# r-mafi/ClaraGenomicsAnalysis

Measured on AMD Instinct MI355X. Metric: POA windows/sec (consensus), higher is better.
Workload: dtype int16

## Files before the change

### claragenomicsanalysis_amd/csrc/poa_batch.cpp

```cpp
#include <claraparabricks/genomeworks/cudapoa/batch.hpp>
#include <claraparabricks/genomeworks/cudapoa/utils.hpp>

#include "gwamd_cudapoa.h"
#include "host_common.hpp"
#include "poa_batch_internal.hpp"
#include "poa_common.hpp"

#include <hip/hip_runtime.h>

#include <algorithm>
#include <cstdio>
#include <cstdlib>
#include <cstring>
#include <iomanip>
#include <sstream>
#include <string>

extern "C" hipError_t gwamd_internal_poa_launch(const gwamd::poa::Buffers* b, const gwamd::poa::Dims* d,
                                       const gwamd::poa::Scores* sc, int score_bits, int size_bits, int banded,
                                       int msa, hipStream_t stream);
extern "C" int gwamd_internal_poa_blocks_per_cu(const gwamd::poa::Dims* d, int score_bits, int size_bits, int banded,
                                                int msa);

namespace claraparabricks
// ... 458 lines not shown
        num_seqs_           = 0;
        next_scores_offset_ = 0;
        avail_scorebuf_     = scorebuf_alloc_;
        generated_          = false;
    }

    int32_t score_bits() const { return score_bits_; }
    int32_t size_bits() const { return size_bits_; }
    const gwamd::poa::Dims& dims() const { return dims_; }
    const std::vector<uint8_t>& host_cons() const { return h_cons_; }
    const std::vector<uint16_t>& host_cov() const { return h_cov_; }
    const std::vector<int32_t>& host_cons_len() const { return h_len_out_; }
    const std::vector<uint8_t>& host_status() const { return h_status_; }
    const std::vector<uint8_t>& host_msa() const { return h_msa_; }
    const std::vector<int32_t>& host_msa_len() const { return h_msa_len_; }
    const std::vector<uint8_t>& host_msa_status() const { return h_msa_status_; }
    const std::vector<uint8_t>& host_g_bases() const { return h_g_bases_; }
    const std::vector<uint16_t>& host_g_in_cnt() const { return h_g_in_cnt_; }
    const std::vector<int32_t>& host_g_in_e() const { return h_g_in_e_; }
    const std::vector<uint16_t>& host_g_in_w() const { return h_g_in_w_; }
    const std::vector<int32_t>& host_final_nodes() const { return h_final_nodes_; }
    int32_t window_num_seqs(int32_t w) const { return h_win_.as<const gwamd::poa::WindowDesc>()[w].num_seqs; }
    int8_t output_mask() const { return output_mask_; }
    int64_t device_bytes() const { return int64_t(d_slab_.n + d_codes_.n + d_seqs_.n + d_wts_.n + d_len_.n + d_off_.n + d_win_.n); }
    int32_t kernel_kind() const
    {
        return dims_.lds_kernel == 3 ? (dims_.band_ad ? 4 : 3) : (dims_.lds_kernel ? 2 : 1);
    }
    int32_t max_poas() const { return max_poas_; }
    int32_t max_sequence_size() const { return bs_.max_sequence_size; }
    int32_t slots() const { return slots_; }
    int32_t resident_slots() const { return blocks_per_cu_; }
    void set_spoa_accurate(bool on) { dims_.spoa_accurate = on ? 1 : 0; }
    bool spoa_accurate() const { return dims_.spoa_accurate != 0; }

    void get_phases(int64_t* out)
    {
        ScopedDevice dev(device_id_);
        if (poa_count_ == 0)
            return;
        GWAMD_HIP_CHECK(hipMemcpyAsync(out, bufs_.phase, size_t(poa_count_) * 8 * gwamd::poa::kPhases,
                                       hipMemcpyDeviceToHost, stream_));
        GWAMD_HIP_CHECK(hipStreamSynchronize(stream_));
    }

    void get_stats(int64_t* cells, int32_t* final_nodes)
    {
        ScopedDevice dev(device_id_);
        if (poa_count_ == 0)
            return;
        GWAMD_HIP_CHECK(hipMemcpyAsync(cells, bufs_.cells, size_t(poa_count_) * 8, hipMemcpyDeviceToHost, stream_));
        GWAMD_HIP_CHECK(hipMemcpyAsync(final_nodes, bufs_.final_nodes, size_t(poa_count_) * 4, hipMemcpyDeviceToHost,
                                       stream_));
        GWAMD_HIP_CHECK(hipStreamSynchronize(stream_));
    }

private:
    int64_t window_bytes(int sz, bool msa) const
    {
        const int64_t mn = dims_.max_nodes, E = gwamd::poa::kMaxEdges, S = dims_.max_seqs;
        int64_t b        = 0;
        b += align8(mn) + 4 * align8(mn * 2) + align8(mn * E * 2);
        b += 3 * align8(mn * E * sz) + 2 * align8(mn * sz);
        b += align8(dims_.max_consensus) + align8(int64_t(dims_.max_consensus) * 2) + 32;
        b += int64_t(S) * dims_.max_seq_len * 2 + S * 12;
        if (msa)
            b += align8(mn * E * S * 2) + align8(mn * E * 2) + align8(S * sz) +
                 align8(S * int64_t(dims_.max_consensus));
        return b;
    }

    int64_t slot_bytes(int sz, int sbytes) const
    {
        const int64_t mn = dims_.max_nodes;
        int64_t b        = 0;
        b += 2 * align8(int64_t(dims_.aln_cap) * sz);
        b += int64_t(dims_.score_rows) * dims_.score_stride * sbytes;
        if (dims_.lds_kernel)
            b += dims_.aux_stride;
        b += align8(mn * 4) + align8(mn * 4 * sz);
        return b;
    }

    void plan_lds_kernel()
    {
        dims_.lds_kernel = 0;
        const char* env  = gwamd::host::diag_env("GWAMD_POA_KERNEL");
        if (env && std::string(env) == "v1")
            return;
        if (banded_ || size_bits_ != 16 || (score_bits_ != 16 && score_bits_ != 32))
            return;
        const bool wide      = score_bits_ == 32;
        auto a16             = [](int64_t v) { return (v + 15) & ~int64_t(15); };
        int ring_rows        = 8;
        const int64_t read_b = a16(int64_t(dims_.max_seq_len) + 48);
        int cpl = 8, nw = 1;
        const int ms = dims_.max_seq_len;
        if (!wide && ms > 512)
            nw = 2;
        if (wide)
        {
            nw  = ms <= 512 ? 1 : (ms <= 1024 ? 2 : (ms <= 2048 ? 4 : 8));
            cpl = ms <= 4096 ? 8 : 16;
        }
        if (const char* sh = gwamd::host::diag_env("GWAMD_POA_LDS_SHAPE"))
        {
            int c = 0, n = 0;
            if (std::sscanf(sh, "%d,%d", &c, &n) == 2)
            {
                const bool known =
                    wide ? ((c == 8 && (n == 1 || n == 2 || n == 4 || n == 8)) || (c == 16 && n == 8))
                         : ((n == 1 && (c == 8 || c == 16 || c == 24 || c == 32)) || (c == 8 && n >= 2 && n <= 4) ||
                            (c == 16 && n == 4) || (c == 4 && n == 4));
                if (!known)
                    throw std::invalid_argument("GWAMD_POA_LDS_SHAPE: unsupported columns/waves pair");
                cpl = c, nw = n;
            }
        }
        const int ebytes     = wide ? 4 : 2;
        const int64_t add_b  = 5 * a16(dims_.max_seq_len + 16) + 2 * (int64_t(dims_.max_nodes) + dims_.max_seq_len);
        const int64_t tile_b = int64_t(gwamd::poa::kTileRows) * gwamd::poa::kTileCols + gwamd::poa::kTbRankBytes;
        const int64_t rec_b  = a16(int64_t(dims_.max_nodes + 2) * 4);
        const int64_t sh_b   = a16(wide ? gwamd::poa::kShBytesW(nw) : gwamd::poa::kShBytes(nw));
        auto ring_bytes      = [&](int rows) {
            return a16(std::max<int64_t>({int64_t(rows) * dims_.score_stride * ebytes, tile_b, add_b}));
        };
        int64_t ring_b       = ring_bytes(ring_rows);
        int64_t fixed        = read_b + ring_b + rec_b + sh_b;
        int64_t target       = 40960 - 16;
        if (wide)
        {
            int64_t chosen = 0;
            for (int64_t budget : {int64_t(81920 - 16), int64_t(163840 - 64)})
            {
                for (int rows : {8, 4})
                {
                    const int64_t rb = ring_bytes(rows);
                    const int64_t fx = read_b + rb + rec_b + sh_b;
                    if (fx + 2048 <= budget)
                    {
                        ring_rows = rows, ring_b = rb, fixed = fx, chosen = budget;
                        break;
                    }
                }
                if (chosen)
                    break;
            }
            if (!chosen)
                return;
            target = chosen;
        }
        int64_t xl_cap       = std::max<int64_t>(1024, (target - fixed) / 2);
        xl_cap               = std::min<int64_t>(xl_cap, 65535);
        int64_t total        = fixed + a16(xl_cap * 2);
        if (const char* pad = gwamd::host::diag_env("GWAMD_POA_LDS_PAD"))
            total += a16(std::atoi(pad));
        if (total > (wide ? 163840 - 64 : 65536))
            return;
        dims_.lds_kernel    = 1;
        dims_.tb_rank       = tb_rank_default();
        dims_.lds_ring_off  = int32_t(read_b);
        dims_.lds_ring_rows = ring_rows;
        dims_.lds_rec_off   = int32_t(read_b + ring_b);
        dims_.lds_xl_off    = int32_t(read_b + ring_b + rec_b);
        dims_.lds_xl_cap    = int32_t(xl_cap);
        dims_.lds_sh_off    = int32_t(read_b + ring_b + rec_b + a16(xl_cap * 2));
        dims_.lds_bytes     = int32_t(total);
        dims_.lds_cpl       = cpl;
        dims_.lds_waves     = nw;
        dims_.code_stride   = int32_t(a16(int64_t(dims_.max_seq_len) + 48));
        const int64_t code_b = int64_t(dims_.score_rows) * dims_.code_stride;
        const int64_t cr_b   = a16(int64_t(dims_.max_nodes + 2) * ebytes);
        dims_.aux_carry_off  = int32_t(code_b);
        dims_.aux_stride     = code_b + cr_b;
    }

public:
    static int tb_rank_default()
    {
        int above_bits = 0;
        if (const char* ab = gwamd::host::diag_env("GWAMD_TB_ABOVE"))
            above_bits = (std::min(std::max(std::atoi(ab), 0), 6) + 1) << 3;
        return tb_walk_bits() | above_bits;
    }
    static int diag_bits()
    {
        const char* r = gwamd::host::diag_env("GWAMD_TOPSORT_RING");
        const char* f = gwamd::host::diag_env("GWAMD_POA_FWD");
        const char* t = gwamd::host::diag_env("GWAMD_TOPSORT");
        const char* d = gwamd::host::diag_env("GWAMD_RACON");
        const char* c = gwamd::host::diag_env("GWAMD_CONSENSUS");
        const char* b = gwamd::host::diag_env("GWAMD_CONSENSUS_LDS_BYTES");
        const int cap = b ? std::min(std::max(std::atoi(b), 1), 65535) : 0;
        return ((r && std::atoi(r) != 0) ? 1 : 0) | ((f && std::string(f) == "v1") ? 2 : 0) |
               ((t && std::string(t) == "fifo") ? 4 : 0) | ((d && std::string(d) == "v1") ? 8 : 0) |
               ((c && std::string(c) == "hbm") ? 16 : 0) | int(uint32_t(cap) << 16);
    }
    static int tb_walk_bits()
    {
        const char* ev = gwamd::host::diag_env("GWAMD_TB_WALK");
        const std::string v = ev ? ev : "";
        if (v == "scalar")
            return 2;
        if (v == "rect")
            return 1;
        if (v == "scalar_rect")
            return 0;
        if (v == "strip32")
            return 7;
        if (v == "scalar_strip32")
            return 6;
        return 3;
    }

private:
    void plan_band_kernel()
    {
        if (!banded_ || dims_.lds_kernel)
            return;
        const char* env = gwamd::host::diag_env("GWAMD_POA_KERNEL");
        if (env && std::string(env) == "v1")
            return;
        const int bw = dims_.band_width;
        if (bw % 128 != 0 || bw < 128 || bw > 1024 || gap_ > 0)
            return;
        auto a16          = [](int64_t v) { return (v + 15) & ~int64_t(15); };
        const int cpl     = bw / 64;
        const int sbytes  = score_bits_ / 8;
        const int rowsz   = (bw + gwamd::poa::kBandPad + cpl + cpl - 1) / cpl * cpl;
        const int64_t ms  = dims_.max_seq_len, mn = dims_.max_nodes;
        const int64_t read_b  = a16(gwamd::poa::kReadGuard + ms + bw + 48);
        const int64_t sh_b    = 64;
        const int ring_rows   = gwamd::poa::band_ring_rows(cpl), tile_rows = gwamd::poa::band_tile_rows(cpl);
        const int64_t ring_b  = a16(int64_t(ring_rows) * rowsz * sbytes) + 4 * 256 * 4 + 1024 * 4;
        const int64_t tile_b  = a16(int64_t(tile_rows) * bw + 64 * 16 + 512 + gwamd::poa::kTbRankBytes);
        const int64_t flags_b = 2 * a16(mn + 2);
        const int64_t add_b   = 7 * a16(ms + 16) + a16(2 * (mn + ms + 16));
        const int64_t ad_b    = a16(int64_t(gwamd::poa::kAdRing) * rowsz * sbytes + gwamd::poa::kWave * sbytes) +
                             a16(mn / 8 + 64);
        const char* fwd_env   = gwamd::host::diag_env("GWAMD_BAND_FWD");
        const bool force_ad   = fwd_env && std::string(fwd_env) == "ad" && cpl <= 4;
        const bool no_ad      = fwd_env && std::string(fwd_env) == "row";
        const int64_t min_w   = std::max({ring_b, tile_b, flags_b, force_ad ? ad_b : int64_t(0)});
        const int64_t want_w  = std::max(min_w, add_b);
        const int64_t kStatic = 256;
        int64_t total         = 0;
        int chosen_per_cu     = 1;
        for (int per_cu : {4, 2, 1})
        {
            const int64_t budget = (163840 / per_cu - kStatic) & ~int64_t(15);
            if ((!force_ad && read_b + want_w + sh_b <= budget) || per_cu == 1)
            {
                total         = budget;
                chosen_per_cu = per_cu;
                break;
            }
        }
        const int64_t work = total - read_b - sh_b;
        if (work < min_w)
            return;
        dims_.lds_kernel     = 3;
        int ad_waves = gwamd::poa::kAdMaxWaves;
        if (const char* ev = gwamd::host::diag_env("GWAMD_BAND_AD_WAVES"))
            ad_waves = std::max(1, std::min(gwamd::poa::kAdMaxWaves, std::atoi(ev)));
        dims_.band_ad        = (!no_ad && cpl <= 4 && chosen_per_cu == 1 && work >= ad_b) ? ad_waves : 0;
        dims_.tb_rank        = tb_rank_default();
        dims_.lds_cpl        = cpl;
        dims_.lds_waves      = 1;
        dims_.lds_bytes      = int32_t(total);
        dims_.lds_ring_off   = int32_t(read_b);
        dims_.lds_ring_rows  = ring_rows;
        dims_.lds_work_bytes = int32_t(work);
        dims_.lds_sh_off     = int32_t(read_b + work);
        dims_.score_stride   = rowsz;
        dims_.code_stride    = bw;
        const int64_t rows   = dims_.score_rows;
        int64_t o            = a16(rows * bw);
// ... 572 lines not shown
                             int32_t* max_nodes)
{
    return guarded([&] {
        batch->impl->fetch_graphs();
        const int32_t n = batch->impl->get_total_poas();
        for (int32_t w = 0; w < n; w++)
        {
            status[w]    = int32_t(batch->impl->graph_status(w));
            num_nodes[w] = batch->impl->host_final_nodes()[w];
        }
        *bases      = batch->impl->host_g_bases().data();
        *in_count   = batch->impl->host_g_in_cnt().data();
        *in_edges   = batch->impl->host_g_in_e().data();
        *in_weights = batch->impl->host_g_in_w().data();
        *max_nodes  = batch->impl->dims().max_nodes;
        return 0;
    });
}

int32_t gwamd_poa_batch_id(const gwamd_poa_batch* batch) { return batch->impl->batch_id(); }

void gwamd_poa_reset(gwamd_poa_batch* batch) { batch->impl->reset(); }

int32_t gwamd_poa_get_stats(gwamd_poa_batch* batch, int64_t* cells, int32_t* final_nodes)
{
    return guarded([&] {
        batch->impl->get_stats(cells, final_nodes);
        return 0;
    });
}

int32_t gwamd_poa_get_phase_ticks(gwamd_poa_batch* batch, int64_t* ticks)
{
    return guarded([&] {
        batch->impl->get_phases(ticks);
        return int32_t(gwamd::poa::kPhases);
    });
}

int32_t gwamd_poa_get_types(const gwamd_poa_batch* batch, int32_t* score_bits, int32_t* size_bits)
{
    *score_bits = batch->impl->score_bits();
    *size_bits  = batch->impl->size_bits();
    return batch->impl->kernel_kind();
}

int32_t gwamd_poa_env_tuning(int32_t* tb_rank, int32_t* band_fwd, int32_t* force_v1, int32_t* diag)
{
    if (!tb_rank || !band_fwd || !force_v1 || !diag)
    {
        gwamd::host::last_error() = "gwamd_poa_env_tuning: NULL output";
        return GWAMD_E_INVALID_ARGUMENT;
    }
    *tb_rank            = claraparabricks::genomeworks::cudapoa::PoaBatch::tb_rank_default();
    const char* fwd     = gwamd::host::diag_env("GWAMD_BAND_FWD");
    *band_fwd           = !fwd ? 0 : (std::string(fwd) == "ad" ? 1 : (std::string(fwd) == "row" ? 2 : 0));
    const char* kern    = gwamd::host::diag_env("GWAMD_POA_KERNEL");
    *force_v1           = kern && std::string(kern) == "v1" ? 1 : 0;
    *diag               = claraparabricks::genomeworks::cudapoa::PoaBatch::diag_bits();
    return 0;
}

int32_t gwamd_poa_set_spoa_accurate(gwamd_poa_batch* batch, int32_t on)
{
    const int32_t was = batch->impl->spoa_accurate() ? 1 : 0;
    batch->impl->set_spoa_accurate(on != 0);
    return was;
}

int32_t gwamd_poa_get_capacity(const gwamd_poa_batch* batch, int64_t* device_bytes, int32_t* max_poas)
{
    *device_bytes = batch->impl->device_bytes();
    *max_poas     = batch->impl->max_poas();
    return 0;
}

int32_t gwamd_poa_get_grid(const gwamd_poa_batch* batch, int32_t* slots, int32_t* resident)
{
    *slots    = batch->impl->slots();
    *resident = batch->impl->resident_slots();
    return 0;
}

static size_t query_free_memory(uint64_t given)
{
    if (given != 0)
        return size_t(given);
    size_t free_mem = 0, total = 0;
    if (hipMemGetInfo(&free_mem, &total) != hipSuccess)
        throw std::runtime_error("hipMemGetInfo failed");
    return free_mem;
}

int64_t gwamd_poa_estimate_max_poas(int32_t max_seq_sz, int32_t max_seq_per_poa, int32_t band_width, int32_t banded,
                                    int32_t msa, uint64_t free_device_memory, float quota, int32_t mismatch,
                                    int32_t gap, int32_t match)
{
    int64_t r = 0;
    const int32_t rc = guarded([&]() -> int32_t {
        r = cp::estimate_max_poas(cp::BatchSize(max_seq_sz, max_seq_per_poa, band_width), banded != 0, msa != 0,
                                  query_free_memory(free_device_memory), quota, mismatch, gap, match);
        return 0;
    });
    return rc != 0 ? int64_t(rc) : r;
}

int32_t gwamd_poa_get_multi_batch_sizes(const int32_t* group_max_len, const int32_t* group_num_reads,
                                        int32_t num_groups, uint64_t free_device_memory, int32_t banded,
                                        int32_t msa, int32_t band_width, const int32_t* bins, int32_t num_bins,
                                        float quota, int32_t mismatch, int32_t gap, int32_t match,
                                        int32_t* num_batches, int32_t* batch_max_seq, int32_t* batch_num_reads,
                                        int32_t* group_batch, int32_t* group_rank)
{
    return guarded([&]() -> int32_t {
        std::vector<cp::Group> groups(size_t(std::max(num_groups, 0)));
        for (int32_t i = 0; i < num_groups; i++)
        {
            groups[i].resize(size_t(std::max(group_num_reads[i], 1)));
            for (auto& e : groups[i])
                e = cp::Entry{nullptr, nullptr, 0};
            groups[i][0].length = group_max_len[i];
        }
        std::vector<int32_t> bin_vec;
        if (bins && num_bins > 0)
            bin_vec.assign(bins, bins + num_bins);
        std::vector<cp::BatchSize> sizes;
        std::vector<std::vector<int32_t>> per_batch;
        cp::get_multi_batch_sizes_for_memory(sizes, per_batch, groups, query_free_memory(free_device_memory),
                                         banded != 0, msa != 0, band_width, bin_vec.empty() ? nullptr : &bin_vec,
                                         quota, mismatch, gap, match);
        *num_batches = int32_t(sizes.size());
        for (size_t b = 0; b < sizes.size(); b++)
        {
            batch_max_seq[b]   = sizes[b].max_sequence_size;
            batch_num_reads[b] = sizes[b].max_sequences_per_poa;
            for (size_t r = 0; r < per_batch[b].size(); r++)
            {
                group_batch[per_batch[b][r]] = int32_t(b);
                group_rank[per_batch[b][r]]  = int32_t(r);
            }
        }
        return 0;
    });
}

}
```

### claragenomicsanalysis_amd/csrc/poa_common.hpp

```cpp
#pragma once

#include <cstdint>

namespace gwamd
{
namespace poa
{

constexpr int kMaxEdges      = 50;
constexpr int kMaxAlignments = 50;
constexpr int kBandPad       = 8;
constexpr int kWave          = 64;
constexpr int kCellsPerLane  = 8;
constexpr int kChunk         = kWave * kCellsPerLane;
constexpr int kAdRing        = 128;
constexpr int kAdSpillDist   = kAdRing - kWave + 1;
constexpr int band_ring_rows(int cpl) { return cpl >= 16 ? 8 : 16; }
constexpr int band_tile_rows(int cpl) { return cpl >= 10 ? 32 : 64; }
constexpr int kReadGuard     = 64;
constexpr int kAdMaxWaves    = 4;
constexpr int kColShift      = 7;

enum Status : uint8_t
{
    kSuccess               = 0,
    kExceededMaxPoas       = 1,
    kExceededMaxSeqSize    = 2,
    kExceededMaxSeqsPerPoa = 3,
    kNodeCountExceeded     = 4,
    kEdgeCountExceeded     = 5,
    kSeqLenExceededNodes   = 6,
    kLoopCountExceeded     = 7,
    kOutputTypeUnavailable = 8,
    kGenericError          = 9,
};

struct WindowDesc
{
    int32_t first_seq;
    int32_t num_seqs;
};

struct Dims
{
    int32_t max_nodes;
    int32_t max_seqs;
    int32_t max_seq_len;
    int32_t max_consensus;
    int32_t score_stride;
    int32_t score_rows;
    int32_t aln_cap;
    int32_t band_width;
    int32_t want_consensus;
    int32_t spoa_accurate;
    int32_t lds_kernel;
    int32_t lds_bytes;
    int32_t lds_ring_off;
    int32_t lds_ring_rows;
    int32_t lds_sh_off;
    int32_t lds_rec_off;
    int32_t lds_xl_off;
    int32_t lds_xl_cap;
    int32_t lds_cpl;
    int32_t lds_waves;
    int32_t code_stride;
    int64_t aux_stride;
    int32_t aux_carry_off;
    int32_t lds_work_bytes;
    int32_t aux_reca_off;
    int32_t aux_recb_off;
    int32_t aux_col0_off;
    int32_t aux_flag_off;
    int32_t aux_xl_off;
    int32_t aux_xl_cap;
    int32_t aux_bx_off;
    int32_t aux_recc_off;
    int32_t aux_rece_off;
    int32_t band_ad;
    int32_t tb_rank;
    int32_t diag;
};

constexpr int kTbRankBytes = 7 * 144 + 128 * 4;

constexpr int kShProg    = 16;
constexpr int kShEnd     = 32;
constexpr int kShBnd     = 64;
constexpr int kShChan    = 128;
constexpr int kChanRows  = 64;
constexpr int kMaxWaves  = 4;
constexpr int kShBytes(int waves) { return kShChan + (waves - 1) * kChanRows * 4; }
constexpr int kShEndW   = 32;
constexpr int kShProgW  = 64;
constexpr int kShBndW   = 128;
constexpr int kShChanW  = 384;
constexpr int kMaxRingW = 8;
constexpr int kShBytesW(int waves) { return kShChanW + (waves - 1) * kChanRows * 8; }

constexpr int kTileRows = 128;
constexpr int kTileCols = 128;
constexpr int kTileXlMin = 512;

struct Buffers
{
    const uint8_t* seqs;
    const int8_t* wts;
    const int32_t* seq_len;
    const int64_t* seq_off;
    const WindowDesc* windows;
    const int32_t* order;
    int32_t num_windows;
    int32_t* head;
    int32_t num_slots;
    uint8_t* base;
    uint16_t* in_cnt;
    uint16_t* out_cnt;
    uint16_t* aln_cnt;
    uint16_t* node_cov;
    uint16_t* in_w;
    void* in_e;
    void* out_e;
    void* aln;
    void* sorted;
    void* pos;
    void* ag;
    void* ar;
    void* scores;
    uint8_t* codes;
    int32_t* cscore;
    void* cpred;
    uint16_t* edge_cov;
    uint16_t* edge_cov_cnt;
    void* seq_begin;
    uint8_t* cons;
    uint16_t* cov;
    int32_t* cons_len;
    uint8_t* status;
    uint8_t* msa_status;
    uint8_t* msa;
    int32_t* msa_len;
    int32_t* final_nodes;
    int64_t* cells;
    int64_t* phase;
};

enum Phase
{
    kPhBackbone = 0,
    kPhForward,
    kPhTraceback,
    kPhAdd,
    kPhTopsort,
    kPhOutput,
    kPhRowProg,
    kPhTotal,
    kPhases
};

struct Scores
{
    int32_t gap, mismatch, match;
};

}
// ... 2 lines not shown
```

### claragenomicsanalysis_amd/csrc/poa_kernels.hip

```cpp
#include <hip/hip_runtime.h>

#include <climits>
#include <cstdint>
#include <type_traits>

#include "poa_wave.hpp"

namespace gwamd
{
namespace poa
{

template <typename ScoreT, typename SizeT, bool BANDED, bool MSA>
__global__ void __launch_bounds__(kWave) poa_window_kernel(Buffers b, Dims d, Scores sc)
{
    extern __shared__ __align__(16) uint8_t lds_read[];
    __shared__ int sh_alen;
    __shared__ int sh_status;
    __shared__ int sh_len;

    const int w = b.order ? b.order[blockIdx.x] : int(blockIdx.x);
    if (w >= b.num_windows)
        return;
    const int lane = threadIdx.x;
// ... 948 lines not shown
                n     = cn;
                loops = cl;
                continue;
            }
        }
        loops++;
        int pi, pj;
        if (i == 0)
        {
            pi = 0;
            pj = j - 1;
        }
        else
        {
            const int cj = j + kColShift;
            if (i < ti0 || i >= ti0 + kTileRows || cj < tj0 || cj >= tj0 + kTileCols)
                load_tile(i, cj);
            const int code_v   = int(tile[(i - ti0) * kTileCols + (cj - tj0)]);
            const int rec_v    = int(prec[i]);
            const int code     = uniform(code_v);
            const uint32_t rec = uint32_t(uniform(rec_v));
            const int dir      = code & 3;
            if (dir == 2)
            {
                pi = i;
                pj = j - 1;
            }
            else
            {
                const int np = int((rec >> 8) & 63), k = code >> 2;
                pi = np == 0 ? 0
                             : (np == 1 ? i - int(rec >> 16)
                                        : (np == int(kRecEscape) ? uniform(pred_row(g, int(g.sorted[i - 1]), k))
                                                                 : uniform(int(pxl[(rec >> 16) + k]))));
                pj = dir == 0 ? j - 1 : j;
            }
        }
        if (lane == (n & (kWave - 1)))
        {
            eg = i == pi ? -1 : i;
            er = j == pj ? -1 : j - 1;
        }
        n++;
        if ((n & (kWave - 1)) == 0)
            flush(n);
        i = pi;
        j = pj;
    }
    if ((n & (kWave - 1)) != 0)
        flush(n);
    wave_sync();
    if (loops >= bound || n > aln_cap)
        return -1;
    return n;
}

#include "poa_fwd2.hpp"
#include "poa_fwd_w.hpp"

template <bool MSA, int CPL, int NW, bool W>
__global__ void __launch_bounds__(kWave * NW, W ? (NW >= 8 ? 2 : 1) : (NW >= 4 ? 2 : 1))
    poa_window_kernel_lds(Buffers b, Dims d, Scores sc)
{
    using SizeT  = int16_t;
    using RowT   = typename std::conditional<W, int32_t, int16_t>::type;
    extern __shared__ __align__(16) uint8_t lds[];
    __shared__ int sh_status;
    __shared__ int sh_len;

    __shared__ int sh_next;
    if (int(blockIdx.x) >= b.num_windows)
        return;
    const int tid      = threadIdx.x;
    const int lane     = tid & (kWave - 1);
    const int wave     = uniform(tid / kWave);
    constexpr int kThr = kWave * NW;
    const size_t slot  = blockIdx.x;

    uint8_t* lread   = lds;
    RowT* ring       = reinterpret_cast<RowT*>(lds + d.lds_ring_off);
    uint8_t* tile    = lds + d.lds_ring_off;
    const int rstride = d.score_stride;
    GWAMD_LDS uint8_t* shb = (GWAMD_LDS uint8_t*)(lds) + d.lds_sh_off;
    AddScratch AX;
    {
        GWAMD_LDS uint8_t* a = (GWAMD_LDS uint8_t*)(lds) + d.lds_ring_off;
        const int ms         = (d.max_seq_len + 16) & ~15;
        AX.gid               = (GWAMD_LDS uint16_t*)(a);
        AX.curr              = (GWAMD_LDS uint16_t*)(a + 2 * ms);
        AX.kind              = a + 4 * ms;
        AX.owner             = (GWAMD_LDS uint16_t*)(a + 5 * ms);
        AX.sh                = (GWAMD_LDS int*)(shb);
    }

    for (int idx = blockIdx.x; idx < b.num_windows;)
    {
    const int w     = b.order ? b.order[idx] : idx;
    const size_t mn = size_t(d.max_nodes);
    WinGraph<SizeT> g;
    g.base      = b.base + w * mn;
    g.in_cnt    = b.in_cnt + w * mn;
    g.out_cnt   = b.out_cnt + w * mn;
    g.aln_cnt   = b.aln_cnt + w * mn;
    g.cov       = b.node_cov + w * mn;
    g.in_w      = b.in_w + w * mn * kMaxEdges;
    g.in_e      = static_cast<SizeT*>(b.in_e) + w * mn * kMaxEdges;
    g.out_e     = static_cast<SizeT*>(b.out_e) + w * mn * kMaxEdges;
    g.aln       = static_cast<SizeT*>(b.aln) + w * mn * kMaxAlignments;
    g.sorted    = static_cast<SizeT*>(b.sorted) + w * mn;
    g.pos       = static_cast<SizeT*>(b.pos) + w * mn;
    g.max_nodes = d.max_nodes;

    SizeT* ag        = static_cast<SizeT*>(b.ag) + slot * d.aln_cap;
    SizeT* ar        = static_cast<SizeT*>(b.ar) + slot * d.aln_cap;
    RowT* spill      = static_cast<RowT*>(b.scores) + slot * d.score_rows * size_t(rstride);
    uint8_t* codes   = b.codes + slot * size_t(d.aux_stride);
    uint32_t* rec    = reinterpret_cast<uint32_t*>(lds + d.lds_rec_off);
    uint16_t* xl     = reinterpret_cast<uint16_t*>(lds + d.lds_xl_off);
    RowT* carry      = reinterpret_cast<RowT*>(codes + d.aux_carry_off);
    RowProg P{rec, xl, d.lds_ring_rows - 1};
    int32_t* cscore  = b.cscore + slot * mn;
    SizeT* cpred     = static_cast<SizeT*>(b.cpred) + slot * mn * 4;
    uint16_t* ecov   = MSA ? b.edge_cov + w * mn * kMaxEdges * d.max_seqs : nullptr;
    uint16_t* ecovc  = MSA ? b.edge_cov_cnt + w * mn * kMaxEdges : nullptr;
    SizeT* seq_begin = MSA ? static_cast<SizeT*>(b.seq_begin) + size_t(w) * d.max_seqs : nullptr;

    PhaseTimer ph;
    FwdProf fp;
#ifdef GWAMD_FWD_PROFILE
    const bool use_v2 = false;
#else
    const bool use_v2 = !W && fwd2_ok(sc) && !(d.diag & 2);
#endif
    const WindowDesc wd = b.windows[w];
    const int nseq      = wd.num_seqs;
    int status          = kSuccess;
    int64_t cells       = 0;
    int node_count      = 0;
    int lv_hint         = 0;

    if (nseq > 0)
    {
        const int len0      = b.seq_len[wd.first_seq];
        const uint8_t* seq0 = b.seqs + b.seq_off[wd.first_seq];
        const int8_t* w0    = b.wts + b.seq_off[wd.first_seq];
        if (wave == 0)
            build_backbone<SizeT, MSA>(g, seq0, w0, len0, lane, ecov, ecovc, seq_begin, d.max_seqs);
        node_count = len0;
        ph.lap<kPhBackbone>();
        for (int s = 1; s < nseq; s++)
        {
            if (node_count >= d.max_nodes)
            {
                status = kNodeCountExceeded;
                break;
            }
            const int L           = b.seq_len[wd.first_seq + s];
            const int64_t off     = b.seq_off[wd.first_seq + s];
            const uint8_t* read_g = b.seqs + off;
            const int8_t* wts_g   = b.wts + off;
            const int padded      = (L + 32 + 15) & ~15;
            for (int j = tid; j < padded; j += kThr)
                lread[j] = j < L ? read_g[j] : 0;
            const int V = node_count;
            if (wave == 0)
                build_row_program<SizeT>(g, V, rec, xl, d.lds_xl_cap, d.lds_ring_rows, lane,
                                         (GWAMD_LDS uint8_t*)(lds) + d.lds_ring_off);
            if (NW > 1)
            {
                constexpr int kP = W ? kShProgW : kShProg;
                constexpr int kB = W ? kShBytesW(NW) : kShBytes(NW);
                for (int t = tid; t < (kB - kP) / 4; t += kThr)
                    reinterpret_cast<GWAMD_LDS int*>(shb + kP)[t] = 0;
            }
            __syncthreads();
            ph.lap<kPhRowProg>();
            cells += int64_t(V + 1) * (L + 1);
            int end_row;
            if constexpr (W)
                end_row = nw_forward_lds_w<CPL, NW, SizeT>(g, P, V, lread, L, ring, rstride, spill, rstride, codes,
                                                           d.code_stride, sc, shb, carry, tid);
            else if constexpr (CPL <= 16)
                end_row = use_v2 ? nw_forward_lds_v2<CPL, NW, SizeT>(g, P, V, lread, L, ring, rstride, spill, rstride,
                                                                     codes, d.code_stride, sc, shb, carry, tid,
                                                                     d.lds_xl_cap)
                                 : nw_forward_lds_pk<CPL, NW, SizeT>(g, P, V, lread, L, ring, rstride, spill, rstride,
                                                                     codes, d.code_stride, sc, shb, carry, tid, fp);
            else
                end_row = nw_forward_lds_pk<CPL, NW, SizeT>(g, P, V, lread, L, ring, rstride, spill, rstride, codes,
                                                            d.code_stride, sc, shb, carry, tid, fp);
            __syncthreads();
            ph.lap<kPhForward>();
            if (wave == 0)
            {
                const int alen_w = traceback_codes<SizeT>(g, P, V, L, end_row, codes, d.code_stride, tile, ag, ar,
                                                          d.aln_cap, lane, (d.tb_rank & 1) != 0,
                                                          d.tb_rank);
                if (lane == 0)
                    sh_len = alen_w;
            }
            __syncthreads();
            const int alen = uniform(sh_len);
            __syncthreads();
            ph.lap<kPhTraceback>();
            if (alen == -1)
            {
                status = kLoopCountExceeded;
                break;
            }
            if (wave == 0)
            {
                int nc = node_count;
                int rc = add_alignment_parallel<SizeT, MSA>(g, nc, ag, ar, alen, L, lread, wts_g, s, ecov, ecovc,
                                                             seq_begin, d.max_seqs, AX, lane);
                if (rc < 0)
                {
                    if (lane == 0)
                    {
                        sh_status = add_alignment<SizeT, MSA>(g, nc, ag, ar, alen, read_g, wts_g, s, ecov, ecovc,
                                                              seq_begin, d.max_seqs);
                        sh_len    = nc;
                    }
                    wave_sync();
                    rc = sh_status;
                    nc = sh_len;
                }
                ph.lap<kPhAdd>();
                if (lane == 0)
                {
                    sh_status = rc;
                    sh_len    = nc;
                }
            }
            __syncthreads();
            int rc       = uniform(sh_status);
            int nc       = uniform(sh_len);
            bool lv_done = false;
            __syncthreads();
            if (rc == kSuccess && !d.spoa_accurate && !(d.diag & 4))
                lv_done = topsort_levels<SizeT, NW>(g, nc, V, (GWAMD_LDS uint8_t*)(lds), d.lds_sh_off, tid, kThr,
                                                    cpred, lv_hint);
            lv_hint = lv_done ? nc : 0;
            if (wave == 0)
            {
                if (rc == kSuccess && !lv_done)
                {
                    if (d.spoa_accurate)
                        rc = topsort_racon_wave<SizeT>(g, nc, cscore, cpred, 4 * d.max_nodes, lane,
                                                       (GWAMD_LDS uint8_t*)(lds), d.lds_sh_off);
                    else if (!topsort_lds<SizeT>(g, nc, (GWAMD_LDS uint8_t*)(lds), d.lds_sh_off, AX.sh, lane, nullptr,
                                                       (d.diag & 1) != 0) &&
                             !topsort_lds_big<SizeT>(g, nc, (GWAMD_LDS uint8_t*)(lds), d.lds_sh_off, lane))
                    {
                        if (lane == 0)
                            topsort_kahn<SizeT>(g, nc, cscore);
                        wave_sync();
                    }
                }
                ph.lap<kPhTopsort>();
                wave_sync();
                if (lane == 0)
                {
                    sh_status = rc;
                    sh_len    = nc;
                }
            }
            __syncthreads();
            status     = uniform(sh_status);
            node_count = uniform(sh_len);
            __syncthreads();
            if (status != kSuccess)
                break;
        }
    }
    if (wave == 0)
    {
        finish_window<SizeT, MSA, NW>(b, d, w, lane, g, status, nseq, node_count, cscore, cpred, ecov, ecovc,
                                      seq_begin, sh_len, sh_status, (GWAMD_LDS uint8_t*)(lds), d.lds_sh_off);
        ph.lap<kPhOutput>();
        if (lane == 0)
        {
            if (b.phase)
            {
                ph.store(b.phase + size_t(w) * kPhases);
#ifdef GWAMD_FWD_PROFILE
                const int slot[8] = {kPhBackbone, kPhAdd, kPhTopsort, kPhOutput, kPhForward, kPhTraceback, kPhRowProg,
                                     kPhTotal};
                for (int i = 0; i < 8; i++)
                    b.phase[size_t(w) * kPhases + slot[i]] = int64_t(fp.t[i]);
#endif
            }
            b.final_nodes[w] = node_count;
            b.cells[w]       = cells;
        }
    }
#if defined(GWAMD_FWD_PROFILE) && defined(GWAMD_FWD_PROFILE_WAVE)
    __syncthreads();
// ... 576 lines not shown
```

### claragenomicsanalysis_amd/csrc/poa_wave.hpp

```cpp
#pragma once

#include <hip/hip_runtime.h>

#include <climits>
#include <cstdint>
#include <type_traits>

#include "poa_device.hpp"

#define GWAMD_LDS __attribute__((address_space(3)))
#define GWAMD_GLB __attribute__((address_space(1)))

#include "poa_consensus.hpp"

namespace gwamd
{
namespace poa
{

template <typename T>
__device__ __forceinline__ GWAMD_LDS T* lds_of(T* p)
{
    return (GWAMD_LDS T*)(uintptr_t)(uint32_t)(uintptr_t)(p);
}
// ... 736 lines not shown
        if (lane == 0)
            X.sh[2 + wv] = err;
        __syncthreads();
        for (int q = 0; q < nwv; q++)
            err = min(err, int(X.sh[2 + q]));
    }
    if (err != INT_MAX)
        return err & 0xff;
    bar();
    lap(5);
    if (wv == 0)
        add_write_new_nodes<SizeT>(g, X, L, read, lane);
    bar();
    lap(6);
    for (int r0 = wv * kAU * kWave; r0 < L; r0 += stepA)
    {
        int curr[kAU], head[kAU], kind[kAU], wsum[kAU], ic[kAU], oc[kAU], cv[kAU], hit[kAU], ohit[kAU];
#pragma unroll
        for (int u = 0; u < kAU; u++)
        {
            const int rp = r0 + u * kWave + lane;
            const bool in = rp < L;
            curr[u]       = in ? int(X.curr[rp]) : 0;
            head[u]       = (in && rp > 0) ? int(X.curr[rp - 1]) : 0;
            kind[u]       = (in && rp > 0) ? int(X.kind[rp]) : -1;
            wsum[u]       = (in && rp > 0) ? int(uint16_t(int(w[rp - 1]))) + int(w[rp]) : 0;
            const int hs  = (in && rp > 0) ? int(X.hit[rp]) : 0xff;
            const int os  = (in && rp > 0) ? int(X.ohit[rp]) : 0xff;
            hit[u]        = hs == 0xff ? -1 : hs;
            ohit[u]       = os == 0xff ? -1 : os;
            if (MSA && in && rp == 0)
                seq_begin[s] = SizeT(curr[u]);
        }
#pragma unroll
        for (int u = 0; u < kAU; u++)
        {
            const int rp  = r0 + u * kWave + lane;
            const bool nw = kind[u] >= 0 && !(kind[u] & 4);
            ic[u]         = nw ? int(g.in_cnt[curr[u]]) : 0;
            oc[u]         = nw ? int(g.out_cnt[head[u]]) : 0;
            cv[u]         = rp < L ? int(g.cov[curr[u]]) : 0;
        }
#pragma unroll
        for (int u = 0; u < kAU; u++)
        {
            const int rp = r0 + u * kWave + lane;
            if (rp >= L)
                continue;
            if (kind[u] >= 0)
            {
                const int cu = curr[u], hd = head[u];
                if (kind[u] & 4)
                {
                    if (hit[u] >= 0)
                        g.in_w[cu * kMaxEdges + hit[u]] = uint16_t(int(g.in_w[cu * kMaxEdges + hit[u]]) + wsum[u]);
                    if (MSA && ohit[u] >= 0)
                    {
                        const int c                                             = int(ecov_cnt[hd * kMaxEdges + ohit[u]]);
                        ecov[size_t(hd * kMaxEdges + ohit[u]) * max_seqs + c] = uint16_t(s);
                        ecov_cnt[hd * kMaxEdges + ohit[u]]                      = uint16_t(c + 1);
                    }
                }
                else
                {
                    g.in_e[cu * kMaxEdges + ic[u]] = SizeT(hd);
                    g.in_w[cu * kMaxEdges + ic[u]] = uint16_t(wsum[u]);
                    g.in_cnt[cu]                   = uint16_t(ic[u] + 1);
                    g.out_e[hd * kMaxEdges + oc[u]] = SizeT(cu);
                    if (MSA)
                    {
                        ecov_cnt[hd * kMaxEdges + oc[u]]                = 1;
                        ecov[size_t(hd * kMaxEdges + oc[u]) * max_seqs] = uint16_t(s);
                    }
                    g.out_cnt[hd] = uint16_t(oc[u] + 1);
                }
            }
            g.cov[curr[u]] = uint16_t(cv[u] + 1);
        }
    }
    node_count = nc0 + nnew;
    bar();
    lap(7);
    return kSuccess;
}

constexpr int kRaconCsrStack = 4096;

template <typename SizeT>
__device__ __forceinline__ bool racon_dfs_csr(WinGraph<SizeT> g, int n, GWAMD_LDS uint8_t* marks,
                                              GWAMD_LDS uint32_t* info, GWAMD_LDS uint16_t* lists,
                                              GWAMD_LDS uint16_t* stack, int cap, int lane, int32_t* heads_,
                                              SizeT* mpos, int* ncols)
{
    GWAMD_GLB int32_t* heads  = (GWAMD_GLB int32_t*)(heads_);
    const uint64_t lt         = (uint64_t(1) << lane) - 1;
    int kq                    = 0;
    int v0                    = 0;
    while (true)
    {
        int id = -1, m = 0;
        uint32_t w = 0;
        for (; v0 < n; v0 += kWave)
        {
            const int v       = v0 + lane;
            const int vc      = v < n ? v : 0;
            const int mr      = int(marks[vc]);
            const uint32_t iw = info[vc];
            const int mk      = v < n ? mr : 2;
            const uint64_t bf = __builtin_amdgcn_ballot_w64((mk & 3) == 0);
            if (bf)
            {
                const int l = __builtin_ctzll(bf);
                id          = v0 + l;
                m           = __builtin_amdgcn_readlane(mk, l);
                w           = uint32_t(__builtin_amdgcn_readlane(int(iw), l));
                break;
            }
        }
        if (id < 0)
            break;
        v0        = id + 1;
        int top   = 0;
        int below = 0;
        if (lane == 0)
            stack[0] = uint16_t(id);
        while (true)
        {
            const int mm = m & 3;
            if (mm == 0)
            {
                const int ic  = int((w >> 20) & 63u);
                const int cnt = ic + ((m & 4) ? int(w >> 26) : 0);
                const int o   = int(w & 0xfffffu);
                const int e0 = lane, e1 = lane + kWave;
                const int l0r = int(lists[e0 < cnt ? o + e0 : 0]);
                const int n0  = e0 < cnt ? l0r : 0;
                const int k0r = int(marks[n0]);
                const uint32_t w0 = info[n0];
                const int k0      = e0 < cnt ? k0r : 2;
                int n1 = 0, k1 = 2;
                uint32_t w1 = 0;
                if (cnt > kWave)
                {
                    n1 = e1 < cnt ? int(lists[o + e1]) : 0;
                    k1 = e1 < cnt ? int(marks[n1]) : 2;
                    w1 = info[n1];
                }
                const bool p0     = (k0 & 3) != 2;
                const bool p1     = (k1 & 3) != 2;
                const uint64_t b0 = __builtin_amdgcn_ballot_w64(p0);
                const uint64_t b1 = __builtin_amdgcn_ballot_w64(p1);
                const int c0 = __popcll(b0), c1 = __popcll(b1);
                if (c0 + c1 != 0)
                {
                    if (top + c0 + c1 >= cap)
                        return false;
                    if (p0)
                    {
                        stack[top + 1 + __popcll(b0 & lt)] = uint16_t(n0);
                        if (e0 >= ic)
                            marks[n0] = uint8_t(k0 & 3);
                    }
                    if (p1)
                    {
                        stack[top + 1 + c0 + __popcll(b1 & lt)] = uint16_t(n1);
                        if (e1 >= ic)
// ... 1395 lines not shown
```

Measured before the change: 17270.

## Run graph add-alignment across all waves via a noinline batched routine

Adds a multi-wave add_alignment_waves path that uses every wave of the block, not only wave 0, to insert the traceback alignment into the POA graph. Extra LDS scratch (hit/ohit/shared words) is carved from the ring region when it fits. The routine reloads its arguments from the kernarg segment, keeping register pressure out of the main kernel. Env flags keep the old wave0 path and a serial path as fallbacks. The risk is the extra call overhead and cross-wave barriers inside the add step.

```diff
diff --git a/claragenomicsanalysis_amd/csrc/poa_batch.cpp b/claragenomicsanalysis_amd/csrc/poa_batch.cpp
--- a/claragenomicsanalysis_amd/csrc/poa_batch.cpp
+++ b/claragenomicsanalysis_amd/csrc/poa_batch.cpp
@@ -564,20 +564,23 @@
         return b;
     }
 
-    void plan_lds_kernel()
-    {
-        dims_.lds_kernel = 0;
+    void plan_lds_kernel() { plan_lds_layout(dims_, banded_, size_bits_, score_bits_); }
+
+public:
+    static void plan_lds_layout(gwamd::poa::Dims& dims, bool banded, int size_bits, int score_bits)
+    {
+        dims.lds_kernel = 0;
         const char* env  = gwamd::host::diag_env("GWAMD_POA_KERNEL");
         if (env && std::string(env) == "v1")
             return;
-        if (banded_ || size_bits_ != 16 || (score_bits_ != 16 && score_bits_ != 32))
+        if (banded || size_bits != 16 || (score_bits != 16 && score_bits != 32))
             return;
-        const bool wide      = score_bits_ == 32;
+        const bool wide      = score_bits == 32;
         auto a16             = [](int64_t v) { return (v + 15) & ~int64_t(15); };
         int ring_rows        = 8;
-        const int64_t read_b = a16(int64_t(dims_.max_seq_len) + 48);
+        const int64_t read_b = gwamd::poa::lds_read_bytes(dims.max_seq_len);
         int cpl = 8, nw = 1;
-        const int ms = dims_.max_seq_len;
+        const int ms = dims.max_seq_len;
         if (!wide && ms > 512)
             nw = 2;
         if (wide)
@@ -600,12 +603,12 @@
             }
         }
         const int ebytes     = wide ? 4 : 2;
-        const int64_t add_b  = 5 * a16(dims_.max_seq_len + 16) + 2 * (int64_t(dims_.max_nodes) + dims_.max_seq_len);
+        const int64_t add_b  = 5 * a16(dims.max_seq_len + 16) + 2 * (int64_t(dims.max_nodes) + dims.max_seq_len);
         const int64_t tile_b = int64_t(gwamd::poa::kTileRows) * gwamd::poa::kTileCols + gwamd::poa::kTbRankBytes;
-        const int64_t rec_b  = a16(int64_t(dims_.max_nodes + 2) * 4);
+        const int64_t rec_b  = a16(int64_t(dims.max_nodes + 2) * 4);
         const int64_t sh_b   = a16(wide ? gwamd::poa::kShBytesW(nw) : gwamd::poa::kShBytes(nw));
         auto ring_bytes      = [&](int rows) {
-            return a16(std::max<int64_t>({int64_t(rows) * dims_.score_stride * ebytes, tile_b, add_b}));
+            return a16(std::max<int64_t>({int64_t(rows) * dims.score_stride * ebytes, tile_b, add_b}));
         };
         int64_t ring_b       = ring_bytes(ring_rows);
         int64_t fixed        = read_b + ring_b + rec_b + sh_b;
@@ -639,22 +642,22 @@
             total += a16(std::atoi(pad));
         if (total > (wide ? 163840 - 64 : 65536))
             return;
-        dims_.lds_kernel    = 1;
-        dims_.tb_rank       = tb_rank_default();
-        dims_.lds_ring_off  = int32_t(read_b);
-        dims_.lds_ring_rows = ring_rows;
-        dims_.lds_rec_off   = int32_t(read_b + ring_b);
-        dims_.lds_xl_off    = int32_t(read_b + ring_b + rec_b);
-        dims_.lds_xl_cap    = int32_t(xl_cap);
-        dims_.lds_sh_off    = int32_t(read_b + ring_b + rec_b + a16(xl_cap * 2));
-        dims_.lds_bytes     = int32_t(total);
-        dims_.lds_cpl       = cpl;
-        dims_.lds_waves     = nw;
-        dims_.code_stride   = int32_t(a16(int64_t(dims_.max_seq_len) + 48));
-        const int64_t code_b = int64_t(dims_.score_rows) * dims_.code_stride;
-        const int64_t cr_b   = a16(int64_t(dims_.max_nodes + 2) * ebytes);
-        dims_.aux_carry_off  = int32_t(code_b);
-        dims_.aux_stride     = code_b + cr_b;
+        dims.lds_kernel    = 1;
+        dims.tb_rank       = tb_rank_default();
+        dims.lds_ring_off  = int32_t(read_b);
+        dims.lds_ring_rows = ring_rows;
+        dims.lds_rec_off   = int32_t(read_b + ring_b);
+        dims.lds_xl_off    = int32_t(read_b + ring_b + rec_b);
+        dims.lds_xl_cap    = int32_t(xl_cap);
+        dims.lds_sh_off    = int32_t(read_b + ring_b + rec_b + a16(xl_cap * 2));
+        dims.lds_bytes     = int32_t(total);
+        dims.lds_cpl       = cpl;
+        dims.lds_waves     = nw;
+        dims.code_stride   = int32_t(a16(int64_t(dims.max_seq_len) + 48));
+        const int64_t code_b = int64_t(dims.score_rows) * dims.code_stride;
+        const int64_t cr_b   = a16(int64_t(dims.max_nodes + 2) * ebytes);
+        dims.aux_carry_off  = int32_t(code_b);
+        dims.aux_stride     = code_b + cr_b;
     }
 
 public:
@@ -673,8 +676,10 @@
         const char* d = gwamd::host::diag_env("GWAMD_RACON");
         const char* c = gwamd::host::diag_env("GWAMD_CONSENSUS");
         const char* b = gwamd::host::diag_env("GWAMD_CONSENSUS_LDS_BYTES");
+        const char* a = gwamd::host::diag_env("GWAMD_POA_ADD");
         const int cap = b ? std::min(std::max(std::atoi(b), 1), 65535) : 0;
-        return ((r && std::atoi(r) != 0) ? 1 : 0) | ((f && std::string(f) == "v1") ? 2 : 0) |
+        const int add = (a && std::string(a) == "wave0") ? 32 : ((a && std::string(a) == "serial") ? 64 : 0);
+        return add | ((r && std::atoi(r) != 0) ? 1 : 0) | ((f && std::string(f) == "v1") ? 2 : 0) |
                ((t && std::string(t) == "fifo") ? 4 : 0) | ((d && std::string(d) == "v1") ? 8 : 0) |
                ((c && std::string(c) == "hbm") ? 16 : 0) | int(uint32_t(cap) << 16);
     }
@@ -1413,6 +1418,44 @@
     return 0;
 }
 
+long long gwamd_internal_poa_lds_add_bytes(int32_t max_seq_len, int32_t max_nodes)
+{
+    return gwamd::poa::lds_add_bytes(max_seq_len, max_nodes);
+}
+
+int32_t gwamd_internal_poa_lds_add_fits(int32_t max_seq_len, int32_t max_nodes, int32_t ring_bytes)
+{
+    return gwamd::poa::lds_add_fits(max_seq_len, max_nodes, ring_bytes) ? 1 : 0;
+}
+
+int32_t gwamd_internal_poa_lds_add_plan(int32_t max_seq_len, int32_t max_nodes, int32_t score_bits,
+                                        int32_t* ring_bytes, int32_t* waves, int32_t* lds_bytes)
+{
+    gwamd::poa::Dims d{};
+    d.max_nodes    = max_nodes;
+    d.max_seq_len  = max_seq_len;
+    d.score_stride = int32_t((int64_t(max_seq_len) + 48 + 7) & ~int64_t(7));
+    d.score_rows   = max_nodes + 2;
+    try
+    {
+        claraparabricks::genomeworks::cudapoa::PoaBatch::plan_lds_layout(d, false, 16, score_bits);
+    }
+    catch (const std::exception& e)
+    {
+        gwamd::host::last_error() = e.what();
+        return -2;
+    }
+    if (!d.lds_kernel)
+        return -1;
+    if (ring_bytes)
+        *ring_bytes = d.lds_rec_off - d.lds_ring_off;
+    if (waves)
+        *waves = d.lds_waves;
+    if (lds_bytes)
+        *lds_bytes = d.lds_bytes;
+    return gwamd::poa::lds_add_fits(d.max_seq_len, d.max_nodes, d.lds_rec_off - d.lds_ring_off) ? 1 : 0;
+}
+
 static size_t query_free_memory(uint64_t given)
 {
     if (given != 0)
diff --git a/claragenomicsanalysis_amd/csrc/poa_common.hpp b/claragenomicsanalysis_amd/csrc/poa_common.hpp
--- a/claragenomicsanalysis_amd/csrc/poa_common.hpp
+++ b/claragenomicsanalysis_amd/csrc/poa_common.hpp
@@ -80,6 +80,28 @@
     int32_t tb_rank;
     int32_t diag;
 };
+
+constexpr int64_t lds_read_bytes(int64_t max_seq_len) { return (max_seq_len + 48 + 15) & ~int64_t(15); }
+
+constexpr int kAddShBytes = 64;
+constexpr int64_t lds_add_ms(int64_t max_seq_len) { return (max_seq_len + 16) & ~int64_t(15); }
+constexpr int64_t lds_add_wave0_bytes(int64_t max_seq_len, int64_t max_nodes)
+{
+    return 5 * lds_add_ms(max_seq_len) + 2 * (max_nodes + max_seq_len);
+}
+constexpr int64_t lds_add_hit_off(int64_t max_seq_len, int64_t max_nodes)
+{
+    return (lds_add_wave0_bytes(max_seq_len, max_nodes) + 15) & ~int64_t(15);
+}
+constexpr int64_t lds_add_bytes(int64_t max_seq_len, int64_t max_nodes)
+{
+    return lds_add_hit_off(max_seq_len, max_nodes) + 2 * lds_add_ms(max_seq_len) + kAddShBytes;
+}
+constexpr bool lds_add_fits(int64_t max_seq_len, int64_t max_nodes, int64_t ring_bytes)
+{
+    return max_seq_len > 0 && max_nodes > 0 && max_nodes + max_seq_len < 65535 &&
+           lds_add_bytes(max_seq_len, max_nodes) <= ring_bytes;
+}
 
 constexpr int kTbRankBytes = 7 * 144 + 128 * 4;
 
diff --git a/claragenomicsanalysis_amd/csrc/poa_kernels.hip b/claragenomicsanalysis_amd/csrc/poa_kernels.hip
--- a/claragenomicsanalysis_amd/csrc/poa_kernels.hip
+++ b/claragenomicsanalysis_amd/csrc/poa_kernels.hip
@@ -1054,16 +1054,10 @@
     uint8_t* tile    = lds + d.lds_ring_off;
     const int rstride = d.score_stride;
     GWAMD_LDS uint8_t* shb = (GWAMD_LDS uint8_t*)(lds) + d.lds_sh_off;
-    AddScratch AX;
-    {
-        GWAMD_LDS uint8_t* a = (GWAMD_LDS uint8_t*)(lds) + d.lds_ring_off;
-        const int ms         = (d.max_seq_len + 16) & ~15;
-        AX.gid               = (GWAMD_LDS uint16_t*)(a);
-        AX.curr              = (GWAMD_LDS uint16_t*)(a + 2 * ms);
-        AX.kind              = a + 4 * ms;
-        AX.owner             = (GWAMD_LDS uint16_t*)(a + 5 * ms);
-        AX.sh                = (GWAMD_LDS int*)(shb);
-    }
+    const AddScratch AX = lds_add_scratch((GWAMD_LDS uint8_t*)(lds) + d.lds_ring_off, d.max_seq_len, d.max_nodes,
+                                          false, (GWAMD_LDS int*)(shb));
+    const bool add_fits = lds_add_fits(d.max_seq_len, d.max_nodes, d.lds_rec_off - d.lds_ring_off);
+    const int add_mode  = (d.diag & 64) ? 2 : (((d.diag & 32) || !add_fits) ? 1 : 0);
 
     for (int idx = blockIdx.x; idx < b.num_windows;)
     {
@@ -1180,11 +1174,23 @@
                 status = kLoopCountExceeded;
                 break;
             }
+            int add_r = -1;
+            if (add_mode == 0)
+                add_r = add_alignment_waves<MSA, NW, NW + (W ? 16 : 0)>(lds_kernel_args(), w, int(slot), s, off,
+                                                                        node_count, alen, L,
+                                                                        (GWAMD_LDS uint8_t*)(lds));
             if (wave == 0)
             {
                 int nc = node_count;
-                int rc = add_alignment_parallel<SizeT, MSA>(g, nc, ag, ar, alen, L, lread, wts_g, s, ecov, ecovc,
-                                                             seq_begin, d.max_seqs, AX, lane);
+                int rc = -1;
+                if (add_mode == 0)
+                {
+                    nc = add_r >> 8;
+                    rc = (add_r & 0xff) == 0xff ? -1 : (add_r & 0xff);
+                }
+                else if (add_mode == 1)
+                    rc = add_alignment_parallel<SizeT, MSA>(g, nc, ag, ar, alen, L, lread, wts_g, s, ecov, ecovc,
+                                                            seq_begin, d.max_seqs, AX, lane);
                 if (rc < 0)
                 {
                     if (lane == 0)
diff --git a/claragenomicsanalysis_amd/csrc/poa_wave.hpp b/claragenomicsanalysis_amd/csrc/poa_wave.hpp
--- a/claragenomicsanalysis_amd/csrc/poa_wave.hpp
+++ b/claragenomicsanalysis_amd/csrc/poa_wave.hpp
@@ -842,6 +842,88 @@
     bar();
     lap(7);
     return kSuccess;
+}
+
+__device__ __forceinline__ AddScratch lds_add_scratch(GWAMD_LDS uint8_t* a, int max_seq_len, int max_nodes, bool waves,
+                                                      GWAMD_LDS int* sh)
+{
+    AddScratch X;
+    const int ms = int(lds_add_ms(max_seq_len));
+    X.gid        = (GWAMD_LDS uint16_t*)(a);
+    X.curr       = (GWAMD_LDS uint16_t*)(a + 2 * ms);
+    X.kind       = a + 4 * ms;
+    X.owner      = (GWAMD_LDS uint16_t*)(a + 5 * ms);
+    X.sh         = sh;
+    if (waves)
+    {
+        const int ho = int(lds_add_hit_off(max_seq_len, max_nodes));
+        X.hit        = a + ho;
+        X.ohit       = a + ho + ms;
+        X.sh         = (GWAMD_LDS int*)(a + ho + 2 * ms);
+    }
+    return X;
+}
+
+struct LdsKernelArgs
+{
+    Buffers b;
+    Dims d;
+    Scores sc;
+};
+static_assert(alignof(Buffers) == 8 && sizeof(Buffers) % 8 == 0 && alignof(Dims) == 8 && sizeof(Dims) % 8 == 0 &&
+                  alignof(Scores) <= 8,
+              "LdsKernelArgs: the kernel's three by-value parameters follow each other without padding");
+typedef const __attribute__((address_space(4))) LdsKernelArgs* LdsKernelArgsPtr;
+__device__ __forceinline__ LdsKernelArgsPtr lds_kernel_args()
+{
+    return (LdsKernelArgsPtr)__builtin_amdgcn_kernarg_segment_ptr();
+}
+
+template <bool MSA, int NW, int kInst = 0>
+__device__ __noinline__ int add_alignment_waves(LdsKernelArgsPtr ka_, int w_, int slot_, int s_, int64_t wts_off,
+                                                int node_count, int alen, int L, GWAMD_LDS uint8_t* lds)
+{
+    using SizeT = int16_t;
+    const uint64_t kav        = uint64_t(uintptr_t(ka_));
+    const LdsKernelArgsPtr ka = (LdsKernelArgsPtr)(uintptr_t(
+        (uint64_t(uint32_t(uniform(int(uint32_t(kav >> 32))))) << 32) | uint32_t(uniform(int(uint32_t(kav))))));
+    const int tid     = int(threadIdx.x);
+    const int lane    = tid & (kWave - 1);
+    const int wv      = NW > 1 ? uniform(tid / kWave) : 0;
+    const size_t w    = size_t(uniform(w_));
+    const size_t slot = size_t(uniform(slot_));
+    const int s       = uniform(s_);
+    const size_t mn   = size_t(ka->d.max_nodes);
+    const int max_seq_len = ka->d.max_seq_len;
+    const int max_seqs    = ka->d.max_seqs;
+    const int64_t woff    = (int64_t(uniform(int(wts_off >> 32))) << 32) | uint32_t(uniform(int(uint32_t(wts_off))));
+    WinGraph<SizeT> g;
+    g.base      = ka->b.base + w * mn;
+    g.in_cnt    = ka->b.in_cnt + w * mn;
+    g.out_cnt   = ka->b.out_cnt + w * mn;
+    g.aln_cnt   = ka->b.aln_cnt + w * mn;
+    g.cov       = ka->b.node_cov + w * mn;
+    g.in_w      = ka->b.in_w + w * mn * kMaxEdges;
+    g.in_e      = static_cast<SizeT*>(ka->b.in_e) + w * mn * kMaxEdges;
+    g.out_e     = static_cast<SizeT*>(ka->b.out_e) + w * mn * kMaxEdges;
+    g.aln       = static_cast<SizeT*>(ka->b.aln) + w * mn * kMaxAlignments;
+    g.sorted    = nullptr;
+    g.pos       = nullptr;
+    g.max_nodes = int(mn);
+    const SizeT* ag  = glb(static_cast<const SizeT*>(ka->b.ag) + slot * ka->d.aln_cap);
+    const SizeT* ar  = glb(static_cast<const SizeT*>(ka->b.ar) + slot * ka->d.aln_cap);
+    const int8_t* wt = glb(ka->b.wts + woff);
+    uint16_t* ecov   = MSA ? glb(ka->b.edge_cov + w * mn * kMaxEdges * max_seqs) : nullptr;
+    uint16_t* ecovc  = MSA ? glb(ka->b.edge_cov_cnt + w * mn * kMaxEdges) : nullptr;
+    SizeT* seq_begin = MSA ? glb(static_cast<SizeT*>(ka->b.seq_begin) + w * max_seqs) : nullptr;
+    lds              = (GWAMD_LDS uint8_t*)(uintptr_t)(uint32_t)uniform(int((uint32_t)(uintptr_t)lds));
+    const AddScratch X =
+        lds_add_scratch(lds + int(lds_read_bytes(max_seq_len)), max_seq_len, int(mn), true, nullptr);
+    int nc       = uniform(node_count);
+    const int rc = add_alignment_parallel_batched<SizeT, MSA, 4>(g, nc, ag, ar, uniform(alen), uniform(L),
+                                                                 (const uint8_t*)(lds), wt, s, ecov, ecovc,
+                                                                 seq_begin, max_seqs, X, lane, nullptr, wv, NW);
+    return (nc << 8) | (rc & 0xff);
 }
 
 constexpr int kRaconCsrStack = 4096;
```

New measurement: 17890, median of 6. 3.6% higher.
